# caishiqing/voice-tts

Hardware: AMD Instinct MI355X
Metric: audio_seconds_per_second (higher is better)
Workload: dtype bf16

## Files before the change

voice-tts_amd/csrc/gpt_kernels.h:

```cpp
#pragma once
#include "common.h"

namespace ixtts {

constexpr int HD = 64;

#ifdef IXTTS_TRACE
constexpr int TRACE_SLOTS = 2048, TRACE_WGS = 512;
static __device__ unsigned long long* g_trace = nullptr;
__device__ __forceinline__ long long clock_after(float dep) {
  long long t;
  asm volatile("s_memrealtime %0\n\ts_waitcnt lgkmcnt(0)" : "=s"(t) : "v"(dep) : "memory");
  return t;
}
struct TraceScope {
  long long t0, ta, tb;
  int kid, seq;
  __device__ __forceinline__ TraceScope(int kernel_id, int launch_seq) : ta(0), tb(0), kid(kernel_id), seq(launch_seq) { t0 = clock_after(0.f); }
  __device__ __forceinline__ void inputs(float dep) { ta = clock_after(dep); }
  __device__ __forceinline__ void mid(float dep) { tb = clock_after(dep); }
  __device__ __forceinline__ void end() {
    const unsigned int blk = blockIdx.x + gridDim.x * (blockIdx.y + gridDim.y * blockIdx.z);
    if (threadIdx.x == 0 && g_trace && blk < TRACE_WGS) {
      const long long t2 = clock_after(0.f);
      unsigned long long* r = g_trace + ((size_t)(seq % TRACE_SLOTS) * TRACE_WGS + blk) * 8;
      r[0] = ((unsigned long long)(kid + 1) << 32) | (unsigned int)seq;
      r[1] = t0; r[2] = ta ? ta : t0; r[3] = tb ? tb : t2; r[4] = t2;
    }
  }
};
#define IXTTS_TRACE_PARAM , int trace_seq
#define IXTTS_TRACE_SEQ trace_seq
#else
struct TraceScope {
  __device__ __forceinline__ TraceScope(int, int) {}
  __device__ __forceinline__ void inputs(float) {}
  __device__ __forceinline__ void mid(float) {}
  __device__ __forceinline__ void end() {}
};
#define IXTTS_TRACE_PARAM
#define IXTTS_TRACE_SEQ 0
#endif

enum { IN_LN = 0, IN_LN2 = 1, IN_PLAIN = 2, IN_ATTN2 = 4, IN_ATTN4 = 5, IN_LN_PART = 6 };
constexpr int MLP_XCDS = 8;

constexpr int PART_STRIDE = 4 + 64;
constexpr int NSPLIT_MAX = 8;
enum { EPI_QKV = 0, EPI_RESID = 1, EPI_GELU = 2, EPI_LOGITS = 3 };

struct GemvArgs {
  const void* wt;
  const float* bias;
  int N;
  int slot0;
  const float* xin;
  int nsplit;
  const float* ln_w;
  const float* ln_b;
  float* out;
  int out_stride;
  void* kcache;
  void* vcache;
  const int* cur_len;
  int smax;
  int heads;
  float* norm_out;
  unsigned* aux;
  float* xout;
  const void* pf_ptr;
  int pf_stride, pf_per, pf_nwaves;
};

#ifndef IXTTS_NT_W
#define IXTTS_NT_W 1
#endif
typedef unsigned int u32x4_t __attribute__((ext_vector_type(4)));
template <bool NT = (IXTTS_NT_W != 0)>
__device__ __forceinline__ uint4 load_w16(const void* p) {
  if constexpr (NT) {
    const u32x4_t v = __builtin_nontemporal_load(reinterpret_cast<const u32x4_t*>(p));
    return make_uint4(v.x, v.y, v.z, v.w);
  } else {
    return *reinterpret_cast<const uint4*>(p);
  }
}
#ifndef IXTTS_PF
#define IXTTS_PF 0
#endif
#if IXTTS_PF > 0
#define IXTTS_PF_PARAM , const void* pf_ptr, int pf_stride, int pf_per, int pf_nwaves
#define IXTTS_PF_ARGS(a) , (a).pf_ptr, (a).pf_stride, (a).pf_per, (a).pf_nwaves
struct PfRegs {
  uint4 r[IXTTS_PF];
};
__device__ __forceinline__ void pf_issue(PfRegs& p, const void* ptr, int stride, int per, int nwaves, int gw, int lane) {
  const char* base = reinterpret_cast<const char*>(ptr) + (size_t)min(gw, nwaves - 1) * stride + lane * 16;
#pragma unroll
  for (int j = 0; j < IXTTS_PF; ++j) p.r[j] = *reinterpret_cast<const uint4*>(base + (size_t)min(j, per - 1) * 1024);
}
__device__ __forceinline__ void pf_retire(const PfRegs& p) {
#pragma unroll
  for (int j = 0; j < IXTTS_PF; ++j) asm volatile("" ::"v"(p.r[j].x), "v"(p.r[j].y), "v"(p.r[j].z), "v"(p.r[j].w));
}
#define IXTTS_PF_ISSUE(gw, lane) PfRegs pf_regs; pf_issue(pf_regs, pf_ptr, pf_stride, pf_per, pf_nwaves, gw, lane); __builtin_amdgcn_sched_barrier(0)
#define IXTTS_PF_RETIRE() pf_retire(pf_regs)
#else
#define IXTTS_PF_PARAM
#define IXTTS_PF_ARGS(a)
#define IXTTS_PF_ISSUE(gw, lane)
#define IXTTS_PF_RETIRE()
#endif

template <typename WT>
struct WVec;
template <>
struct WVec<float> {
  static constexpr int VEC = 4;
  __device__ static __forceinline__ void unpack(const uint4& r, float (&w)[4]) {
    w[0] = __uint_as_float(r.x); w[1] = __uint_as_float(r.y); w[2] = __uint_as_float(r.z); w[3] = __uint_as_float(r.w);
  }
};
template <>
struct WVec<bf16> {
  static constexpr int VEC = 8;
  __device__ static __forceinline__ void unpack(const uint4& v, float (&w)[8]) {
    w[0] = lo_bf16(v.x); w[1] = hi_bf16(v.x); w[2] = lo_bf16(v.y); w[3] = hi_bf16(v.y);
    w[4] = lo_bf16(v.z); w[5] = hi_bf16(v.z); w[6] = lo_bf16(v.w); w[7] = hi_bf16(v.w);
  }
};
template <>
struct WVec<f16> {
  static constexpr int VEC = 8;
  __device__ static __forceinline__ void unpack(const uint4& v, float (&w)[8]) { unpack8<f16>(v, w); }
};

__device__ __forceinline__ void store_kv(float* p, float v) { *p = v; }
__device__ __forceinline__ void store_kv(bf16* p, float v) { *p = __float2bfloat16(v); }
__device__ __forceinline__ void store_kv(f16* p, float v) { *p = f16_sat(v); }

__device__ __forceinline__ float gelu_new_f(float x) {
  const float c = 0.7978845608028654f;
  return 0.5f * x * (1.0f + tanhf(c * (x + 0.044715f * x * x * x)));
}

template <int K, int ROWS, int B, int EPI, typename KVT>
__device__ __forceinline__ void gemv_epilogue(const GemvArgs& a, int lane, int unit, const float (&tot)[ROWS][B],
                                              float pre_bias, float pre_res, int pre_pos) {
  if (lane < ROWS * B) {
    const int r = lane / B, b = lane % B;
    float mine = 0.f;
#pragma unroll
    for (int rr = 0; rr < ROWS; ++rr)
#pragma unroll
      for (int bb = 0; bb < B; ++bb)
        if (rr == r && bb == b) mine = tot[rr][bb];
    const int n = unit * ROWS + r;
    if (n < a.N) {
      const int slot = a.slot0 + b;
      const float v = mine + pre_bias;
      if constexpr (EPI == EPI_RESID) {
        a.out[(size_t)slot * a.out_stride + n] = pre_res + v;
      } else if constexpr (EPI == EPI_GELU) {
        a.out[(size_t)slot * a.out_stride + n] = gelu_new_f(v);
      } else if constexpr (EPI == EPI_LOGITS) {
        a.out[(size_t)slot * a.out_stride + n] = v;
      } else {
        constexpr int D = K;
        if (n < D) {
          a.out[(size_t)slot * a.out_stride + n] = v;
        } else {
          const int which = n / D;
          const int c = n - which * D;
          const int hh = c / HD, d = c % HD;
          KVT* cache = reinterpret_cast<KVT*>(which == 1 ? a.kcache : a.vcache);
          store_kv(cache + (((size_t)slot * a.heads + hh) * a.smax + pre_pos) * HD + d, v);
        }
      }
    }
  }
}

typedef float f32x2 __attribute__((ext_vector_type(2)));

template <typename WT>
__device__ __forceinline__ void unpack2(const uint4& r, f32x2 (&w)[WVec<WT>::VEC / 2]);
template <>
__device__ __forceinline__ void unpack2<float>(const uint4& r, f32x2 (&w)[2]) {
  w[0] = f32x2{__uint_as_float(r.x), __uint_as_float(r.y)};
  w[1] = f32x2{__uint_as_float(r.z), __uint_as_float(r.w)};
}
template <>
__device__ __forceinline__ void unpack2<bf16>(const uint4& r, f32x2 (&w)[4]) {
  w[0] = f32x2{lo_bf16(r.x), hi_bf16(r.x)};
  w[1] = f32x2{lo_bf16(r.y), hi_bf16(r.y)};
  w[2] = f32x2{lo_bf16(r.z), hi_bf16(r.z)};
  w[3] = f32x2{lo_bf16(r.w), hi_bf16(r.w)};
}
template <>
__device__ __forceinline__ void unpack2<f16>(const uint4& r, f32x2 (&w)[4]) {
  w[0] = f32x2{lo_f16(r.x), hi_f16(r.x)};
  w[1] = f32x2{lo_f16(r.y), hi_f16(r.y)};
  w[2] = f32x2{lo_f16(r.z), hi_f16(r.z)};
  w[3] = f32x2{lo_f16(r.w), hi_f16(r.w)};
}

template <int B, int WPB>
__device__ __forceinline__ void block_sum(float (&s)[B], float* red, int wave, int lane) {
#pragma unroll
  for (int b = 0; b < B; ++b) {
    const float t = wave_sum63(s[b]);
    if (lane == 63) red[wave * B + b] = t;
  }
  __syncthreads();
#pragma unroll
  for (int b = 0; b < B; ++b) {
    float t = 0.f;
#pragma unroll
    for (int w = 0; w < WPB; ++w) t += red[w * B + b];
    s[b] = t;
  }
}

template <typename WT, int K, int ROWS, int UNITS, int B, int INP, int EPI, typename KVT, int WPB = 4, bool XLDS = false>
__global__ __launch_bounds__(64 * WPB) void gemv_reg_kernel(const void* wt, const float* xin, const float* bias, float* out, int N, int slot0, int out_stride, int smax,
                                                        void* kcache, void* vcache, const int* cur_len, int heads, int nsplit,
                                                        const float* ln_w, const float* ln_b, unsigned* aux, float* xout IXTTS_PF_PARAM IXTTS_TRACE_PARAM) {
  GemvArgs a;
  a.wt = wt; a.xin = xin; a.bias = bias; a.out = out; a.N = N; a.slot0 = slot0; a.out_stride = out_stride; a.smax = smax;
  a.kcache = kcache; a.vcache = vcache; a.cur_len = cur_len; a.heads = heads; a.nsplit = nsplit; a.ln_w = ln_w; a.ln_b = ln_b;
  a.norm_out = nullptr;
  if (aux != nullptr && blockIdx.x == 0 && threadIdx.x < MLP_XCDS) aux[threadIdx.x * 32] = 0u;
  TraceScope trace(EPI, IXTTS_TRACE_SEQ);
  constexpr int VEC = WVec<WT>::VEC;
  constexpr int PER = 64 * VEC;
  constexpr int NL = ROWS * K / PER;
  static_assert(ROWS * K % PER == 0, "unit must be a whole number of wave loads");
  static_assert(K % VEC == 0 && K % 4 == 0, "row length must be a multiple of the vector width");
  static_assert(XLDS || INP == IN_PLAIN, "LayerNorm / split-S merge inputs are staged by the workgroup (XLDS)");
  constexpr int NSP = INP == IN_ATTN2 ? 2 : (INP == IN_ATTN4 ? 4 : 1);
  constexpr int NPASS = (INP == IN_LN || INP == IN_LN_PART) ? 1 : (INP == IN_LN2 ? 2 : 0);

  const int lane = threadIdx.x & 63;
  const int wave = threadIdx.x >> 6;
  const int unit0 = (blockIdx.x * WPB + wave) * UNITS;
  const int n_units = (a.N + ROWS - 1) / ROWS;
  if (!XLDS && unit0 >= n_units) return;

  constexpr int K4 = K / 4, X4 = B * K4, NT = 64 * WPB, XV = (X4 + NT - 1) / NT;
  f32x2 xr[B][NL][VEC / 2];
  float4 xs4[XLDS ? XV : 1];
  float4 lw4[NPASS == 2 ? XV : 1], lb4[NPASS == 2 ? XV : 1];
  float4 pbias4[INP == IN_LN_PART ? XV : 1], ppart4[INP == IN_LN_PART ? XV : 1][MLP_XCDS];
  float2 pml[NSP > 1 ? XV : 1][NSP];
  float4 pac[NSP > 1 ? XV : 1][NSP];
  if constexpr (XLDS && NSP == 1) {
    const float* xbase = a.xin + (size_t)a.slot0 * K;
#pragma unroll
    for (int i = 0; i < XV; ++i) {
      const int idx = min((int)threadIdx.x + i * NT, X4 - 1);
      xs4[i] = *reinterpret_cast<const float4*>(xbase + (size_t)idx * 4);
      if constexpr (NPASS == 2) {
        lw4[i] = *reinterpret_cast<const float4*>(a.ln_w + (idx % K4) * 4);
        lb4[i] = *reinterpret_cast<const float4*>(a.ln_b + (idx % K4) * 4);
      }
      if constexpr (INP == IN_LN_PART) {
        const int b = idx / K4, k0 = (idx % K4) * 4;
        pbias4[i] = *reinterpret_cast<const float4*>(a.ln_b + k0);
#pragma unroll
        for (int x = 0; x < MLP_XCDS; ++x)
          ppart4[i][x] = *reinterpret_cast<const float4*>(a.ln_w + ((size_t)x * a.nsplit + a.slot0 + b) * K + k0);
      }
    }
  } else if constexpr (XLDS) {
    constexpr int H = K / HD;
#pragma unroll
    for (int i = 0; i < XV; ++i) {
      const int idx = min((int)threadIdx.x + i * NT, X4 - 1);
      const int b = idx / K4, k0 = (idx % K4) * 4;
      const float* p = a.xin + ((size_t)((a.slot0 + b) * H + k0 / HD) * NSP) * PART_STRIDE;
#pragma unroll
      for (int sp = 0; sp < NSP; ++sp) {
        pml[i][sp] = *reinterpret_cast<const float2*>(p + sp * PART_STRIDE);
        pac[i][sp] = *reinterpret_cast<const float4*>(p + sp * PART_STRIDE + 4 + k0 % HD);
      }
    }
  } else {
#pragma unroll
    for (int b = 0; b < B; ++b) {
      const float* xs = a.xin + (size_t)(a.slot0 + b) * K;
#pragma unroll
      for (int j = 0; j < NL; ++j) {
        const int k0 = (j * PER + lane * VEC) % K;
#pragma unroll
        for (int v4 = 0; v4 < VEC / 4; ++v4) {
          const float4 t = *reinterpret_cast<const float4*>(xs + k0 + v4 * 4);
          xr[b][j][v4 * 2] = f32x2{t.x, t.y};
          xr[b][j][v4 * 2 + 1] = f32x2{t.z, t.w};
        }
      }
    }
  }
  __builtin_amdgcn_sched_barrier(0);
  float pre_bias[UNITS], pre_res[UNITS];
  int pre_pos = 0;
  const int elane = min(lane, ROWS * B - 1);
#pragma unroll
  for (int u = 0; u < UNITS; ++u) {
    const int n = min((unit0 + u) * ROWS + elane / B, a.N - 1);
    pre_bias[u] = a.bias[n];
    pre_res[u] = 0.f;
    if constexpr (EPI == EPI_RESID) pre_res[u] = a.out[(size_t)(a.slot0 + elane % B) * a.out_stride + n];
  }
  if constexpr (EPI == EPI_QKV) pre_pos = a.cur_len[a.slot0 + elane % B];
  __builtin_amdgcn_sched_barrier(0);
  uint4 wraw[UNITS][NL];
#pragma unroll
  for (int u = 0; u < UNITS; ++u) {
    const int unit_c = min(unit0 + u, n_units - 1);
    const WT* base = reinterpret_cast<const WT*>(a.wt) + (size_t)unit_c * ROWS * K;
#pragma unroll
    for (int j = 0; j < NL; ++j) {
      const int e = j * PER + lane * VEC;
      wraw[u][j] = load_w16(base + (e < min(ROWS, a.N - unit_c * ROWS) * K ? e : 0));
    }
  }
  __builtin_amdgcn_sched_barrier(0);
  IXTTS_PF_ISSUE(blockIdx.x * WPB + wave, lane);
  if constexpr (XLDS) {
    __shared__ __attribute__((aligned(16))) float xsh[B * K];
    __shared__ float red[(NPASS > 0 ? 2 * NPASS : 1) * WPB * B];
    if constexpr (NSP > 1) {
#pragma unroll
      for (int i = 0; i < XV; ++i) {
        float M = -INFINITY;
#pragma unroll
        for (int sp = 0; sp < NSP; ++sp) M = fmaxf(M, pml[i][sp].x);
        float L = 0.f;
        float4 o = make_float4(0.f, 0.f, 0.f, 0.f);
#pragma unroll
        for (int sp = 0; sp < NSP; ++sp) {
          const float w = (pml[i][sp].x > -INFINITY) ? expf(pml[i][sp].x - M) : 0.f;
          L = fmaf(pml[i][sp].y, w, L);
          o.x = fmaf(pac[i][sp].x, w, o.x); o.y = fmaf(pac[i][sp].y, w, o.y);
          o.z = fmaf(pac[i][sp].z, w, o.z); o.w = fmaf(pac[i][sp].w, w, o.w);
        }
        const float inv = 1.0f / L;
        xs4[i] = make_float4(o.x * inv, o.y * inv, o.z * inv, o.w * inv);
      }
    }
    if constexpr (INP == IN_LN_PART) {
#pragma unroll
      for (int i = 0; i < XV; ++i) {
        float4 t = xs4[i];
        t.x += pbias4[i].x; t.y += pbias4[i].y; t.z += pbias4[i].z; t.w += pbias4[i].w;
#pragma unroll
        for (int x = 0; x < MLP_XCDS; ++x) {
          t.x += ppart4[i][x].x; t.y += ppart4[i][x].y; t.z += ppart4[i][x].z; t.w += ppart4[i][x].w;
        }
        xs4[i] = t;
        const int idx = threadIdx.x + i * NT;
        if (blockIdx.x == 0 && (X4 % NT == 0 || idx < X4))
          *reinterpret_cast<float4*>(xout + (size_t)a.slot0 * K + (size_t)idx * 4) = t;
      }
    }
#pragma unroll
    for (int pass = 0; pass < NPASS; ++pass) {
      float s[B], q[B];
#pragma unroll
      for (int b = 0; b < B; ++b) s[b] = 0.f;
#pragma unroll
      for (int i = 0; i < XV; ++i) {
        const int idx = threadIdx.x + i * NT;
        const int sl = (X4 % NT == 0 || idx < X4) ? idx / K4 : B;
        const float v = (xs4[i].x + xs4[i].y) + (xs4[i].z + xs4[i].w);
#pragma unroll
        for (int b = 0; b < B; ++b) s[b] += (sl == b) ? v : 0.f;
      }
      block_sum<B, WPB>(s, red + (2 * pass) * WPB * B, wave, lane);
#pragma unroll
      for (int b = 0; b < B; ++b) {
        s[b] *= (1.0f / K);
        q[b] = 0.f;
      }
#pragma unroll
      for (int i = 0; i < XV; ++i) {
        const int idx = threadIdx.x + i * NT;
        const int sl = (X4 % NT == 0 || idx < X4) ? idx / K4 : B;
        float mean = 0.f;
#pragma unroll
        for (int b = 0; b < B; ++b) mean = (sl == b) ? s[b] : mean;
        xs4[i].x -= mean; xs4[i].y -= mean; xs4[i].z -= mean; xs4[i].w -= mean;
        const float v = fmaf(xs4[i].x, xs4[i].x, xs4[i].y * xs4[i].y) + fmaf(xs4[i].z, xs4[i].z, xs4[i].w * xs4[i].w);
#pragma unroll
        for (int b = 0; b < B; ++b) q[b] += (sl == b) ? v : 0.f;
      }
      block_sum<B, WPB>(q, red + (2 * pass + 1) * WPB * B, wave, lane);
#pragma unroll
      for (int b = 0; b < B; ++b) q[b] = 1.0f / sqrtf(q[b] * (1.0f / K) + 1e-5f);
#pragma unroll
      for (int i = 0; i < XV; ++i) {
        const int idx = threadIdx.x + i * NT;
        const int sl = (X4 % NT == 0 || idx < X4) ? idx / K4 : B;
        float rstd = 0.f;
#pragma unroll
        for (int b = 0; b < B; ++b) rstd = (sl == b) ? q[b] : rstd;
        xs4[i].x *= rstd; xs4[i].y *= rstd; xs4[i].z *= rstd; xs4[i].w *= rstd;
        if (NPASS == 2 && pass == 0) {
          xs4[i].x = fmaf(xs4[i].x, lw4[i].x, lb4[i].x); xs4[i].y = fmaf(xs4[i].y, lw4[i].y, lb4[i].y);
          xs4[i].z = fmaf(xs4[i].z, lw4[i].z, lb4[i].z); xs4[i].w = fmaf(xs4[i].w, lw4[i].w, lb4[i].w);
        }
      }
    }
#pragma unroll
    for (int i = 0; i < XV; ++i) {
      const int idx = threadIdx.x + i * NT;
      if (X4 % NT == 0 || idx < X4) *reinterpret_cast<float4*>(xsh + idx * 4) = xs4[i];
    }
    __syncthreads();
#pragma unroll
    for (int b = 0; b < B; ++b)
#pragma unroll
      for (int j = 0; j < NL; ++j) {
        const int k0 = (j * PER + lane * VEC) % K;
#pragma unroll
        for (int v4 = 0; v4 < VEC / 4; ++v4) {
          const float4 t = *reinterpret_cast<const float4*>(xsh + b * K + k0 + v4 * 4);
          xr[b][j][v4 * 2] = f32x2{t.x, t.y};
          xr[b][j][v4 * 2 + 1] = f32x2{t.z, t.w};
        }
      }
  }
  trace.inputs(xr[0][0][0].x);
#pragma unroll
  for (int u = 0; u < UNITS; ++u) {
    const int unit = unit0 + u;
    if (unit >= n_units) break;
    const int rows_here = min(ROWS, a.N - unit * ROWS);
    float acc[ROWS][B];
#pragma unroll
    for (int r = 0; r < ROWS; ++r)
#pragma unroll
      for (int b = 0; b < B; ++b) acc[r][b] = 0.f;
#pragma unroll
    for (int j = 0; j < NL; ++j) {
      const int e = j * PER + lane * VEC;
      const int row = (e < rows_here * K) ? e / K : ROWS;
      f32x2 w2[VEC / 2];
      unpack2<WT>(wraw[u][j], w2);
#pragma unroll
      for (int b = 0; b < B; ++b) {
        f32x2 d2 = w2[0] * xr[b][j][0];
#pragma unroll
        for (int v = 1; v < VEC / 2; ++v) d2 = __builtin_elementwise_fma(w2[v], xr[b][j][v], d2);
        const float d = d2.x + d2.y;
#pragma unroll
        for (int r = 0; r < ROWS; ++r) acc[r][b] += (row == r) ? d : 0.f;
      }
    }
    float tot[ROWS][B];
#pragma unroll
    for (int r = 0; r < ROWS; ++r)
#pragma unroll
      for (int b = 0; b < B; ++b) tot[r][b] = wave_sum(acc[r][b]);
    if (u == UNITS - 1) trace.mid(tot[0][0]);
    gemv_epilogue<K, ROWS, B, EPI, KVT>(a, lane, unit, tot, pre_bias[u], pre_res[u], pre_pos);
  }
  IXTTS_PF_RETIRE();
  trace.end();
}

template <typename WT, int K, int ROWS, int UNITS, int B, int EPI, typename KVT, int WPB = 4>
__global__ __launch_bounds__(64 * WPB) void gemv_lds_kernel(const void* wt, const float* xin, const float* bias, float* out, int N, int slot0, int out_stride, int smax,
                                                        void* kcache, void* vcache, const int* cur_len, int heads, int nsplit,
                                                        const float* ln_w, const float* ln_b, unsigned* aux, float* xout IXTTS_PF_PARAM IXTTS_TRACE_PARAM) {
  GemvArgs a;
  a.wt = wt; a.xin = xin; a.bias = bias; a.out = out; a.N = N; a.slot0 = slot0; a.out_stride = out_stride; a.smax = smax;
  a.kcache = kcache; a.vcache = vcache; a.cur_len = cur_len; a.heads = heads; a.nsplit = nsplit; a.ln_w = ln_w; a.ln_b = ln_b;
  a.norm_out = nullptr;
  TraceScope trace(4, IXTTS_TRACE_SEQ);
  constexpr int VEC = WVec<WT>::VEC;
  constexpr int PER = 64 * VEC;
  constexpr int NL = ROWS * K / PER;
  static_assert(ROWS * K % PER == 0, "unit must be a whole number of wave loads");
  extern __shared__ __attribute__((aligned(16))) float xs[];

  const int lane = threadIdx.x & 63;
  const int wave = threadIdx.x >> 6;
  const int unit0 = (blockIdx.x * WPB + wave) * UNITS;
  const int n_units = (a.N + ROWS - 1) / ROWS;

  constexpr int TOT4 = B * K / 4;
  constexpr int NT = 64 * WPB;
  constexpr int XV = (TOT4 + NT - 1) / NT;
  const float* xbase = a.xin + (size_t)a.slot0 * K;
  float4 xv[XV];
#pragma unroll
  for (int i = 0; i < XV; ++i) {
    const int idx = threadIdx.x + i * NT;
    xv[i] = (TOT4 % NT == 0 || idx < TOT4) ? *reinterpret_cast<const float4*>(xbase + (size_t)idx * 4) : make_float4(0.f, 0.f, 0.f, 0.f);
  }
  __builtin_amdgcn_sched_barrier(0);
  float pre_bias[UNITS], pre_res[UNITS];
  const int elane = min(lane, ROWS * B - 1);
#pragma unroll
  for (int u = 0; u < UNITS; ++u) {
    const int n = min((unit0 + u) * ROWS + elane / B, a.N - 1);
    pre_bias[u] = a.bias[n];
    pre_res[u] = 0.f;
    if constexpr (EPI == EPI_RESID) pre_res[u] = a.out[(size_t)(a.slot0 + elane % B) * a.out_stride + n];
  }
  __builtin_amdgcn_sched_barrier(0);
  uint4 wraw[UNITS][NL];
#pragma unroll
  for (int u = 0; u < UNITS; ++u) {
    const int unit = unit0 + u;
    const int unit_c = min(unit, n_units - 1);
    const WT* base = reinterpret_cast<const WT*>(a.wt) + (size_t)unit_c * ROWS * K;
#pragma unroll
    for (int j = 0; j < NL; ++j) {
      const int e = j * PER + lane * VEC;
      wraw[u][j] = load_w16(base + (e < min(ROWS, a.N - unit_c * ROWS) * K ? e : 0));
    }
  }
  __builtin_amdgcn_sched_barrier(0);
  IXTTS_PF_ISSUE(blockIdx.x * WPB + wave, lane);
#pragma unroll
  for (int i = 0; i < XV; ++i) {
    const int idx = threadIdx.x + i * NT;
    if (TOT4 % NT == 0 || idx < TOT4) *reinterpret_cast<float4*>(xs + idx * 4) = xv[i];
  }
  __syncthreads();
  trace.inputs(xv[0].x);

#pragma unroll
  for (int u = 0; u < UNITS; ++u) {
    const int unit = unit0 + u;
    if (unit >= n_units) break;
    float acc[ROWS][B];
#pragma unroll
    for (int r = 0; r < ROWS; ++r)
#pragma unroll
      for (int b = 0; b < B; ++b) acc[r][b] = 0.f;
    const int rows_here = min(ROWS, a.N - unit * ROWS);
#pragma unroll
    for (int j = 0; j < NL; ++j) {
      const int e = j * PER + lane * VEC;
      const int row0 = e / K;
      const int k0 = e - row0 * K;
      const int row = (e < rows_here * K) ? row0 : ROWS;
      float wv[VEC];
      WVec<WT>::unpack(wraw[u][j], wv);
#pragma unroll
      for (int b = 0; b < B; ++b) {
        const float* x = xs + b * K + k0;
        float d = 0.f;
#pragma unroll
        for (int v4 = 0; v4 < VEC / 4; ++v4) {
          const float4 t = *reinterpret_cast<const float4*>(x + v4 * 4);
          d = fmaf(wv[v4 * 4 + 0], t.x, d);
          d = fmaf(wv[v4 * 4 + 1], t.y, d);
          d = fmaf(wv[v4 * 4 + 2], t.z, d);
          d = fmaf(wv[v4 * 4 + 3], t.w, d);
        }
#pragma unroll
        for (int r = 0; r < ROWS; ++r) acc[r][b] += (row == r) ? d : 0.f;
      }
    }
    float tot[ROWS][B];
#pragma unroll
    for (int r = 0; r < ROWS; ++r)
#pragma unroll
      for (int b = 0; b < B; ++b) tot[r][b] = wave_sum(acc[r][b]);
    if (u == UNITS - 1) trace.mid(tot[0][0]);
    gemv_epilogue<K, ROWS, B, EPI, KVT>(a, lane, unit, tot, pre_bias[u], pre_res[u], 0);
  }
  IXTTS_PF_RETIRE();
  trace.end();
}

constexpr int MLP_D = 1280, MLP_FF = 5120, MLP_WAVES = 5, MLP_SLICE = MLP_FF / MLP_XCDS, MLP_ROWS_OUT = MLP_D / 32, MLP_KSUB = MLP_SLICE / MLP_WAVES;
static_assert(MLP_SLICE == 640 && MLP_ROWS_OUT == 40 && MLP_KSUB == 128, "partition of the fused MLP");
constexpr unsigned MLP_SPIN_MAX = 1u << 15;
constexpr int MLP_CTR_STRIDE = MLP_XCDS * 32;

__device__ __forceinline__ float group_sum16(float v) {
  v += dpp_take<0xB1, 0xf, 0xf>(v);
  v += dpp_take<0x4E, 0xf, 0xf>(v);
  v += dpp_take<0x141, 0xf, 0xf>(v);
  v += dpp_take<0x140, 0xf, 0xf>(v);
  return v;
}

__device__ __forceinline__ unsigned xcc_id() {
  unsigned v;
  asm volatile("s_getreg_b32 %0, hwreg(HW_REG_XCC_ID)" : "=s"(v));
  return v & 0xf;
}

static __global__ void mlp_repack_pr_kernel(const bf16* __restrict__ in, bf16* __restrict__ out) {
  const size_t i = (size_t)blockIdx.x * blockDim.x + threadIdx.x;
  constexpr size_t G = (size_t)MLP_XCDS * MLP_D * MLP_SLICE / 8;
  if (i >= G) return;
  const size_t e = i * 8;
  const int c = (int)(e % MLP_SLICE);
  const int n = (int)((e / MLP_SLICE) % MLP_D);
  const int x = (int)(e / ((size_t)MLP_SLICE * MLP_D));
  reinterpret_cast<uint4*>(out)[i] = *reinterpret_cast<const uint4*>(in + (size_t)n * MLP_FF + (size_t)x * MLP_SLICE + c);
}

static __global__ void mlp_xcc_probe_kernel(unsigned* map) {
  if (threadIdx.x == 0) map[blockIdx.x] = xcc_id();
}

template <int B>
__global__ __launch_bounds__(64 * MLP_WAVES) void mlp_fused_kernel(const bf16* __restrict__ wfc, const float* __restrict__ hin, const float* __restrict__ bfc,
                                                                   float* ff, const bf16* __restrict__ wprx, float* __restrict__ part,
                                                                   unsigned* ctr, unsigned* mark, int slot0, int slots) {
  constexpr int K = MLP_D, ROWS = 2, UNITS = 2, VEC = 8, PER = 64 * VEC, NL = ROWS * K / PER, WPB = MLP_WAVES, NT = 64 * WPB;
  constexpr int K4 = K / 4, X4 = B * K4, XV = (X4 + NT - 1) / NT;
  constexpr int NPR = MLP_ROWS_OUT / 4;
  __shared__ __attribute__((aligned(16))) float xsh[B * K];
  __shared__ float red[2 * WPB * B];
  __shared__ float prs[WPB][MLP_ROWS_OUT][B];
  const int lane = threadIdx.x & 63, wave = threadIdx.x >> 6;
  const int xcd = (int)xcc_id() & 7, j = blockIdx.x >> 3;
#ifdef IXTTS_MLP_LOG
  const unsigned long long t_entry = wall_clock64();
  unsigned long long t_ff = 0, t_arrive = 0, t_rel = 0;
  const bool logging = ctr == mark - (size_t)(gridDim.y + 13) * MLP_CTR_STRIDE;
#endif
  const int unit0 = ((xcd * 32 + j) * WPB + wave) * UNITS;

  float4 xs4[XV];
  const float* xbase = hin + (size_t)slot0 * K;
#pragma unroll
  for (int i = 0; i < XV; ++i) {
    const int idx = min((int)threadIdx.x + i * NT, X4 - 1);
    xs4[i] = *reinterpret_cast<const float4*>(xbase + (size_t)idx * 4);
  }
  __builtin_amdgcn_sched_barrier(0);
  float pre_bias[UNITS];
  const int elane = min(lane, ROWS * B - 1);
#pragma unroll
  for (int u = 0; u < UNITS; ++u) pre_bias[u] = bfc[(unit0 + u) * ROWS + elane / B];
  __builtin_amdgcn_sched_barrier(0);
  uint4 wraw[UNITS][NL];
#pragma unroll
  for (int u = 0; u < UNITS; ++u) {
    const bf16* base = wfc + (size_t)(unit0 + u) * ROWS * K;
#pragma unroll
    for (int jj = 0; jj < NL; ++jj) wraw[u][jj] = *reinterpret_cast<const uint4*>(base + jj * PER + lane * VEC);
  }
  __builtin_amdgcn_sched_barrier(0);
  {
    float s[B], q[B];
#pragma unroll
    for (int b = 0; b < B; ++b) s[b] = 0.f;
#pragma unroll
    for (int i = 0; i < XV; ++i) {
      const int idx = threadIdx.x + i * NT;
      const int sl = (X4 % NT == 0 || idx < X4) ? idx / K4 : B;
      const float v = (xs4[i].x + xs4[i].y) + (xs4[i].z + xs4[i].w);
#pragma unroll
      for (int b = 0; b < B; ++b) s[b] += (sl == b) ? v : 0.f;
    }
    block_sum<B, WPB>(s, red, wave, lane);
#pragma unroll
    for (int b = 0; b < B; ++b) {
      s[b] *= (1.0f / K);
      q[b] = 0.f;
    }
#pragma unroll
    for (int i = 0; i < XV; ++i) {
      const int idx = threadIdx.x + i * NT;
      const int sl = (X4 % NT == 0 || idx < X4) ? idx / K4 : B;
      float mean = 0.f;
#pragma unroll
      for (int b = 0; b < B; ++b) mean = (sl == b) ? s[b] : mean;
      xs4[i].x -= mean; xs4[i].y -= mean; xs4[i].z -= mean; xs4[i].w -= mean;
      const float v = fmaf(xs4[i].x, xs4[i].x, xs4[i].y * xs4[i].y) + fmaf(xs4[i].z, xs4[i].z, xs4[i].w * xs4[i].w);
#pragma unroll
      for (int b = 0; b < B; ++b) q[b] += (sl == b) ? v : 0.f;
    }
    block_sum<B, WPB>(q, red + WPB * B, wave, lane);
#pragma unroll
    for (int b = 0; b < B; ++b) q[b] = 1.0f / sqrtf(q[b] * (1.0f / K) + 1e-5f);
#pragma unroll
    for (int i = 0; i < XV; ++i) {
      const int idx = threadIdx.x + i * NT;
      const int sl = (X4 % NT == 0 || idx < X4) ? idx / K4 : B;
      float rstd = 0.f;
#pragma unroll
      for (int b = 0; b < B; ++b) rstd = (sl == b) ? q[b] : rstd;
      xs4[i].x *= rstd; xs4[i].y *= rstd; xs4[i].z *= rstd; xs4[i].w *= rstd;
      if (X4 % NT == 0 || idx < X4) *reinterpret_cast<float4*>(xsh + idx * 4) = xs4[i];
    }
  }
  __syncthreads();
  uint4 praw[NPR];
  {
    const bf16* base = wprx + ((size_t)xcd * MLP_D + (size_t)j * MLP_ROWS_OUT + (lane >> 4)) * MLP_SLICE + wave * MLP_KSUB + (lane & 15) * VEC;
#pragma unroll
    for (int i = 0; i < NPR; ++i) praw[i] = *reinterpret_cast<const uint4*>(base + (size_t)(4 * i) * MLP_SLICE);
  }
  __builtin_amdgcn_sched_barrier(0);
  {
    f32x2 xr[B][NL][VEC / 2];
#pragma unroll
    for (int b = 0; b < B; ++b)
#pragma unroll
      for (int jj = 0; jj < NL; ++jj) {
        const int k0 = (jj * PER + lane * VEC) % K;
#pragma unroll
        for (int v4 = 0; v4 < VEC / 4; ++v4) {
          const float4 t = *reinterpret_cast<const float4*>(xsh + b * K + k0 + v4 * 4);
          xr[b][jj][v4 * 2] = f32x2{t.x, t.y};
          xr[b][jj][v4 * 2 + 1] = f32x2{t.z, t.w};
        }
      }
#pragma unroll
    for (int u = 0; u < UNITS; ++u) {
      float acc[ROWS][B];
#pragma unroll
      for (int r = 0; r < ROWS; ++r)
#pragma unroll
        for (int b = 0; b < B; ++b) acc[r][b] = 0.f;
#pragma unroll
      for (int jj = 0; jj < NL; ++jj) {
        const int row = (jj * PER + lane * VEC) / K;
        f32x2 w2[VEC / 2];
        unpack2<bf16>(wraw[u][jj], w2);
#pragma unroll
        for (int b = 0; b < B; ++b) {
          f32x2 d2 = w2[0] * xr[b][jj][0];
#pragma unroll
          for (int v = 1; v < VEC / 2; ++v) d2 = __builtin_elementwise_fma(w2[v], xr[b][jj][v], d2);
          const float d = d2.x + d2.y;
#pragma unroll
          for (int r = 0; r < ROWS; ++r) acc[r][b] += (row == r) ? d : 0.f;
        }
      }
      float mine = 0.f;
#pragma unroll
      for (int r = 0; r < ROWS; ++r)
#pragma unroll
        for (int b = 0; b < B; ++b) {
          const float t = wave_sum(acc[r][b]);
          mine = (lane == r * B + b) ? t : mine;
        }
      if (lane < ROWS * B) {
        const int r = lane / B, b = lane % B;
        ff[(size_t)(slot0 + b) * MLP_FF + (unit0 + u) * ROWS + r] = gelu_new_f(mine + pre_bias[u]);
      }
    }
  }
#ifdef IXTTS_MLP_LOG
  t_ff = wall_clock64();
#endif
  asm volatile("s_waitcnt vmcnt(0)" ::: "memory");
// ... 1084 lines not shown
```

Measured before the change: 41.13.

## Remap GEMV weight lanes so each wave chunk reuses one activation register slice

Adds a RegMap that assigns each weight load to a fixed row and K-chunk, so activation registers are sized by K/PER chunks instead of per-load. This cuts activation register usage and loads, and removes the per-row select chain in accumulation. A half-wave split handles tails where K is an odd multiple of half a wave load. The LDS reduction read in block_sum is also rotated per batch to avoid bank conflicts. The trade-off is that weight access per lane is no longer fully contiguous across rows.

Result: faster. 41.86, median of 6 (+1.8%).

```diff
diff --git a/voice-tts_amd/csrc/gpt_kernels.h b/voice-tts_amd/csrc/gpt_kernels.h
--- a/voice-tts_amd/csrc/gpt_kernels.h
+++ b/voice-tts_amd/csrc/gpt_kernels.h
@@ -205,7 +205,32 @@
   w[3] = f32x2{lo_f16(r.w), hi_f16(r.w)};
 }
 
-template <int B, int WPB>
+#ifndef IXTTS_XMAP
+#define IXTTS_XMAP 1
+#endif
+template <int K, int ROWS, int VEC>
+struct RegMap {
+  static constexpr int PER = 64 * VEC;
+  static constexpr int NL = ROWS * K / PER;
+  static constexpr int NF = K / PER;
+  static constexpr bool TAIL = K % PER != 0;
+  static constexpr bool XMAP = IXTTS_XMAP != 0 && K >= PER && (!TAIL || (K % PER == PER / 2 && ROWS % 2 == 0));
+  static constexpr int NFR = ROWS * NF;
+  static constexpr int NX = XMAP ? NF + (TAIL ? 1 : 0) : NL;
+  static_assert(!XMAP || NFR + (TAIL ? ROWS / 2 : 0) == NL, "every element of the unit is loaded once");
+  __device__ static constexpr int chunk(int j) { return XMAP ? (j < NFR ? j % NF : NF) : j; }
+  __device__ static constexpr int xk(int c, int lane) {
+    return XMAP ? (c < NF ? c * PER + lane * VEC : NF * PER + (lane & 31) * VEC) : (c * PER + lane * VEC) % K;
+  }
+  __device__ static constexpr int row(int j, int lane) {
+    return XMAP ? (j < NFR ? j / NF : 2 * (j - NFR) + (lane >> 5)) : (j * PER + lane * VEC) / K;
+  }
+  __device__ static constexpr int elem(int j, int lane) {
+    return XMAP ? row(j, lane) * K + xk(chunk(j), lane) : j * PER + lane * VEC;
+  }
+};
+
+template <int B, int WPB, int WSHIFT = 0>
 __device__ __forceinline__ void block_sum(float (&s)[B], float* red, int wave, int lane) {
 #pragma unroll
   for (int b = 0; b < B; ++b) {
@@ -217,7 +242,7 @@
   for (int b = 0; b < B; ++b) {
     float t = 0.f;
 #pragma unroll
-    for (int w = 0; w < WPB; ++w) t += red[w * B + b];
+    for (int w = 0; w < WPB; ++w) t += red[((w + b * WSHIFT) % WPB) * B + b];
     s[b] = t;
   }
 }
@@ -233,8 +258,10 @@
   if (aux != nullptr && blockIdx.x == 0 && threadIdx.x < MLP_XCDS) aux[threadIdx.x * 32] = 0u;
   TraceScope trace(EPI, IXTTS_TRACE_SEQ);
   constexpr int VEC = WVec<WT>::VEC;
-  constexpr int PER = 64 * VEC;
-  constexpr int NL = ROWS * K / PER;
+  using Map = RegMap<K, ROWS, VEC>;
+  constexpr int PER = Map::PER;
+  constexpr int NL = Map::NL;
+  constexpr int NX = Map::NX;
   static_assert(ROWS * K % PER == 0, "unit must be a whole number of wave loads");
   static_assert(K % VEC == 0 && K % 4 == 0, "row length must be a multiple of the vector width");
   static_assert(XLDS || INP == IN_PLAIN, "LayerNorm / split-S merge inputs are staged by the workgroup (XLDS)");
@@ -248,7 +275,8 @@
   if (!XLDS && unit0 >= n_units) return;
 
   constexpr int K4 = K / 4, X4 = B * K4, NT = 64 * WPB, XV = (X4 + NT - 1) / NT;
-  f32x2 xr[B][NL][VEC / 2];
+  constexpr int WSHIFT = K4 % 64 == 0 ? (K4 / 64) % WPB : 0;
+  f32x2 xr[B][NX][VEC / 2];
   float4 xs4[XLDS ? XV : 1];
   float4 lw4[NPASS == 2 ? XV : 1], lb4[NPASS == 2 ? XV : 1];
   float4 pbias4[INP == IN_LN_PART ? XV : 1], ppart4[INP == IN_LN_PART ? XV : 1][MLP_XCDS];
@@ -290,8 +318,8 @@
     for (int b = 0; b < B; ++b) {
       const float* xs = a.xin + (size_t)(a.slot0 + b) * K;
 #pragma unroll
-      for (int j = 0; j < NL; ++j) {
-        const int k0 = (j * PER + lane * VEC) % K;
+      for (int j = 0; j < NX; ++j) {
+        const int k0 = Map::xk(j, lane);
 #pragma unroll
         for (int v4 = 0; v4 < VEC / 4; ++v4) {
           const float4 t = *reinterpret_cast<const float4*>(xs + k0 + v4 * 4);
@@ -321,7 +349,7 @@
     const WT* base = reinterpret_cast<const WT*>(a.wt) + (size_t)unit_c * ROWS * K;
 #pragma unroll
     for (int j = 0; j < NL; ++j) {
-      const int e = j * PER + lane * VEC;
+      const int e = Map::elem(j, lane);
       wraw[u][j] = load_w16(base + (e < min(ROWS, a.N - unit_c * ROWS) * K ? e : 0));
     }
   }
@@ -377,7 +405,7 @@
 #pragma unroll
         for (int b = 0; b < B; ++b) s[b] += (sl == b) ? v : 0.f;
       }
-      block_sum<B, WPB>(s, red + (2 * pass) * WPB * B, wave, lane);
+      block_sum<B, WPB, WSHIFT>(s, red + (2 * pass) * WPB * B, wave, lane);
 #pragma unroll
       for (int b = 0; b < B; ++b) {
         s[b] *= (1.0f / K);
@@ -395,7 +423,7 @@
 #pragma unroll
         for (int b = 0; b < B; ++b) q[b] += (sl == b) ? v : 0.f;
       }
-      block_sum<B, WPB>(q, red + (2 * pass + 1) * WPB * B, wave, lane);
+      block_sum<B, WPB, WSHIFT>(q, red + (2 * pass + 1) * WPB * B, wave, lane);
 #pragma unroll
       for (int b = 0; b < B; ++b) q[b] = 1.0f / sqrtf(q[b] * (1.0f / K) + 1e-5f);
 #pragma unroll
@@ -421,8 +449,8 @@
 #pragma unroll
     for (int b = 0; b < B; ++b)
 #pragma unroll
-      for (int j = 0; j < NL; ++j) {
-        const int k0 = (j * PER + lane * VEC) % K;
+      for (int j = 0; j < NX; ++j) {
+        const int k0 = Map::xk(j, lane);
 #pragma unroll
         for (int v4 = 0; v4 < VEC / 4; ++v4) {
           const float4 t = *reinterpret_cast<const float4*>(xsh + b * K + k0 + v4 * 4);
@@ -444,18 +472,29 @@
       for (int b = 0; b < B; ++b) acc[r][b] = 0.f;
 #pragma unroll
     for (int j = 0; j < NL; ++j) {
-      const int e = j * PER + lane * VEC;
-      const int row = (e < rows_here * K) ? e / K : ROWS;
+      const int xc = Map::chunk(j);
       f32x2 w2[VEC / 2];
       unpack2<WT>(wraw[u][j], w2);
 #pragma unroll
       for (int b = 0; b < B; ++b) {
-        f32x2 d2 = w2[0] * xr[b][j][0];
-#pragma unroll
-        for (int v = 1; v < VEC / 2; ++v) d2 = __builtin_elementwise_fma(w2[v], xr[b][j][v], d2);
+        f32x2 d2 = w2[0] * xr[b][xc][0];
+#pragma unroll
+        for (int v = 1; v < VEC / 2; ++v) d2 = __builtin_elementwise_fma(w2[v], xr[b][xc][v], d2);
         const float d = d2.x + d2.y;
-#pragma unroll
-        for (int r = 0; r < ROWS; ++r) acc[r][b] += (row == r) ? d : 0.f;
+        if constexpr (Map::XMAP) {
+          if (j < Map::NFR) {
+            acc[j / Map::NF][b] += d;
+          } else {
+            const int t = j - Map::NFR;
+            acc[2 * t][b] += (lane < 32) ? d : 0.f;
+            acc[2 * t + 1][b] += (lane < 32) ? 0.f : d;
+          }
+        } else {
+          const int e = Map::elem(j, lane);
+          const int row = (e < rows_here * K) ? e / K : ROWS;
+#pragma unroll
+          for (int r = 0; r < ROWS; ++r) acc[r][b] += (row == r) ? d : 0.f;
+        }
       }
     }
     float tot[ROWS][B];
```
